# halajun/diasss

Measured on AMD Instinct MI355X. Metric: sonar frames/sec end-to-end (extract+match+LM solve), higher is better.
Workload: dtype u8/int32 (extract, match) + f64 (geo gate, LM); 1 GPU; 200 synthetic 2000x1024 frames, dense all-pairs; frames=200, pings=2000, bins=1024, pairs=19900

## Files before the change

diasss_amd/csrc/dsss_pg.hip:

```cpp
#include "dsss_internal.h"
#include "dsss_lm.h"
#include <utility>
#include "dsss_pg_kernels.h"
#include <algorithm>
#include <numeric>
#include <random>
#include <cstdlib>
#include <chrono>
#include <thread>
#include <mutex>
#include <future>

namespace {

struct pg_dev {
    dsss_ctx* ctx = nullptr;
    int rc = DSSS_OK;
    static constexpr size_t CHUNK = (size_t)256 << 20;
    template <typename T> int alloc(dsss_ctx* c, T** p, size_t n) { void* q = nullptr; if (!rc) rc = grab(c, &q, std::max<size_t>(n, 1) * sizeof(T)); *p = (T*)q; return rc; }
    int grab(dsss_ctx* c, void** p, size_t n) {
        if (!ctx) { ctx = c; c->pg_chunk_cur = 0; c->pg_chunk_off = 0; }
        const size_t bytes = (n + 255) & ~(size_t)255;
        for (;;) {
            if (c->pg_chunk_cur < c->pg_chunks.size()) {
// ... 541 lines not shown
        for (const pg_sched* H : { &A.SO, &A.SI })
            for (int l = 0; l < H->nlev; ++l) {
                const int nit = H->lv_ptr[l + 1] - H->lv_ptr[l];
                if (nit > 0) c->pg_last_levels.insert(c->pg_last_levels.end(), { nit, H->max_w6[l], H->max_rows[l], H == &A.SI ? 1 : 0 });
            }
        dv.alloc(c, &d_Tinv, (size_t)std::max(S.npanels, 1) * PG_NB4 * 16);
        size_t need = 0;
        for (const pg_sched* H : { &A.SO, &A.SI })
            for (int l = 0; l < H->nlev; ++l)
                if (64 * H->trsm_chunks[l] > PG_BWD_SPLIT) need = std::max(need, (size_t)(H->lv_ptr[l + 1] - H->lv_ptr[l]) * ((64 * H->trsm_chunks[l] + PG_BWD_RC - 1) / PG_BWD_RC) * 96);
        if ((need > 0 && dv.alloc(c, &d_bwp, need)) || dv.rc) return dv.rc;
        bwd_lds = (int)(((PG_PW * 6) * PG_BWD2_LD + PG_NB4 * 16 + 10 * (PG_PW * 6) + std::min(max_n6, PG_BWD2_SX) + 16) * sizeof(double));
        if (bwd_lds > 160 * 1024) DSSS_FAIL(c, DSSS_E_CAPACITY, "front of %d scalar rows: back-substitution needs %d B of LDS", max_n6, bwd_lds);
        hipFuncSetAttribute((const void*)pg_front_bwd2_kernel, hipFuncAttributeMaxDynamicSharedMemorySize, 160 * 1024);
        (void)hipGetLastError();
        return DSSS_OK;
    }

    void run_levels(const pg_sched& H, const dsched& Dv, int part = 0) {
        for (int l = 0; l < H.nlev; ++l) {
            const int nas = part == 2 ? 0 : H.asmrow_ptr[l + 1] - H.asmrow_ptr[l], nit = part == 1 ? 0 : H.lv_ptr[l + 1] - H.lv_ptr[l], ntl = H.tile_ptr[l + 1] - H.tile_ptr[l];
            const int* itf = Dv.lv_front + H.lv_ptr[l]; const int* its = Dv.lv_step + H.lv_ptr[l];
            if (nas > 0) { dsss_scope s2(c, DSSS_K_PG_ASM);
                hipLaunchKernelGGL(pg_front_asm_kernel, dim3(nas), dim3(256), 0, st, Dv.asm_front + H.asmrow_ptr[l], Dv.asm_row + H.asmrow_ptr[l], d_FD, d_CH, d_rel, d_xr_ptr, d_xr_child, d_xr_row,
                                   d_fa_rowptr, d_fa_src, d_fa_col, d_fa_tr, d_aval, d_x, d_F, d_R); }
            if (nit == 0) continue;
            { dsss_scope s3(c, DSSS_K_PG_DIAG, H.fl_diag[l]);
              hipLaunchKernelGGL(pg_front_diag4_kernel, dim3(nit), dim3(256), 0, st, itf, its, d_FD, d_F, d_R, d_fail, d_Tinv); }
            if (ntl > 0 && ntl <= PG_RSU_MAX_TILES) {
                dsss_scope s45(c, DSSS_K_PG_RSU, H.fl_trsm[l] + H.fl_syrk[l]);
                if (ntl <= PG_RSU32_MAX_TILES)
                    hipLaunchKernelGGL(pg_front_rsu_kernel<32>, dim3(4 * ntl), dim3(256), 0, st, itf, its, d_FD, Dv.tile_item + H.tile_ptr[l], Dv.tile_ij + H.tile_ptr[l], d_F, d_FL, d_R, d_Tinv);
                else hipLaunchKernelGGL(pg_front_rsu_kernel<64>, dim3(ntl), dim3(512), 0, st, itf, its, d_FD, Dv.tile_item + H.tile_ptr[l], Dv.tile_ij + H.tile_ptr[l], d_F, d_FL, d_R, d_Tinv);
            } else if (H.trsm_chunks[l] > 0) {
                { dsss_scope s4(c, DSSS_K_PG_TRSM, H.fl_trsm[l]);
                  hipLaunchKernelGGL(pg_front_trsm2_kernel, dim3(nit, H.trsm_chunks[l]), dim3(256), 0, st, itf, its, d_FD, d_F, d_R, d_Tinv); }
                { dsss_scope s5(c, DSSS_K_PG_ACC, H.fl_syrk[l]);
                  if (ntl > 0) hipLaunchKernelGGL(pg_front_syrk_kernel, dim3(ntl), dim3(256), 0, st, itf, its, d_FD, Dv.tile_item + H.tile_ptr[l], Dv.tile_ij + H.tile_ptr[l], d_F); }
            }
        }
    }
    void run_levels_bwd(const pg_sched& H, const dsched& Dv) {
        for (int l = H.nlev - 1; l >= 0; --l) {
            const int nit = H.lv_ptr[l + 1] - H.lv_ptr[l];
            if (nit == 0) continue;
            dsss_scope s6(c, DSSS_K_PG_BWD, H.fl_bwd[l], 2);
            const int ntl = H.tile_ptr[l + 1] - H.tile_ptr[l];
            const double* Fl = (ntl > 0 && ntl <= PG_RSU_MAX_TILES) ? d_FL : d_F;
// ... 388 lines not shown
```

diasss_amd/csrc/dsss_pg_fronts.hip:

```cpp
#include "dsss_pg_kernels.h"
#include "dsss_pg_dev.h"
#include <utility>
#pragma clang fp contract(fast)

__global__ __launch_bounds__(256) void pg_front_asm_kernel(const int* __restrict__ it_front, const int* __restrict__ it_row, const pg_front* __restrict__ FD,
                                                           const pg_child* __restrict__ CH, const int* __restrict__ rel, const int* __restrict__ xr_ptr,
                                                           const int* __restrict__ xr_child, const int* __restrict__ xr_row, const int* __restrict__ fa_rowptr,
                                                           const int* __restrict__ fa_src, const int* __restrict__ fa_col, const int* __restrict__ fa_tr,
                                                           const double* __restrict__ aval, const double* __restrict__ x, double* __restrict__ F, double* __restrict__ R)
{
    const pg_front fd = FD[it_front[blockIdx.x]];
    const int Rb = it_row[blockIdx.x], ld = fd.ld;
    double* __restrict__ A = F + fd.off + (size_t)(6 * Rb) * ld; double* __restrict__ r = R + fd.roff + 6 * Rb;
    const int ncol = 6 * (Rb + 1);
    for (int cc = threadIdx.x; cc < ncol; cc += 256) {
#pragma unroll
        for (int a = 0; a < 6; ++a) A[(size_t)a * ld + cc] = 0.0;
    }
    if (threadIdx.x < 6) { const int i = 6 * Rb + threadIdx.x; r[threadIdx.x] = i < fd.s6 ? x[(size_t)fd.c0 * 6 + i] : 0.0; }
    __syncthreads();
    {
        const int lo = fa_rowptr[fd.rowptr + Rb], hi = fa_rowptr[fd.rowptr + Rb + 1];
        const int grp = threadIdx.x / 36, el = threadIdx.x % 36;
        if (grp < 7)
            for (int e = lo + grp; e < hi; e += 7) {
                if (e > lo && fa_col[e - 1] == fa_col[e]) continue;
                const int a = el / 6, b = el % 6;
                double v = 0;
                for (int e2 = e; e2 < hi && fa_col[e2] == fa_col[e]; ++e2) v += aval[(size_t)fa_src[e2] * 36 + (fa_tr[e2] ? b * 6 + a : a * 6 + b)];
                A[(size_t)a * ld + fa_col[e] * 6 + b] += v;
            }
    }
    __syncthreads();
    const int q_lo = xr_ptr[fd.rowptr + Rb], q_hi = xr_ptr[fd.rowptr + Rb + 1];
    pg_child cd_n = {}; int i_n = 0;
    if (q_lo < q_hi) { cd_n = CH[xr_child[q_lo]]; i_n = xr_row[q_lo]; }
    for (int q = q_lo; q < q_hi; ++q) {
// ... 88 lines not shown
#pragma unroll
        for (int u = 0; u < 12; ++u) {
            const int e = threadIdx.x + 256 * u, rr = e / 48, c2 = e - 48 * rr;
            *reinterpret_cast<double2*>(&sB[rr * PG_SYRK_LD + 2 * c2]) = v[u];
        }
    }
    const int i0 = 64 * ti + 16 * wave;
    const int ir = i0 + (l & 15);
    double a[24];
    pg_d4 acc[4];
    {
        const double* __restrict__ Ai = A + (size_t)(P.row0 + min(ir, nrows - 1)) * ld + P.col0;
#pragma unroll
        for (int ks = 0; ks < 24; ++ks) { const int k = 4 * ks + (l >> 4); a[ks] = (ir < nrows && k < n) ? Ai[k] : 0.0; }
        pg_strip_load<64>(acc, A, P, true, i0, tj, l);
    }
#pragma unroll
    for (int ks = 0; ks < 24; ++ks) a[ks] = -a[ks];
    __syncthreads();
    if (i0 >= nrows) return;
    pg_strip_update<64>(acc, [&](int ks) { return a[ks]; }, sB, A, P, i0, tj, l);
}

#define PG_LDS_BARRIER() do { asm volatile("s_waitcnt lgkmcnt(0)" ::: "memory"); __builtin_amdgcn_s_barrier(); asm volatile("" ::: "memory"); } while (0)
struct pg_d4_lds { double lp[3][7][64]; double li[2][16]; int bad; };
struct pg_lag_desc { int kind, I, T2; };
constexpr pg_lag_desc pg_lag_get(int W, int NT, int R, int want)
{
    const int I0 = W, I1 = W + 4, K = 4 * NT;
    const bool act0 = I0 < NT, act1 = I1 < 7 && (I1 < NT || I1 == 6);
    int idx = 0;
    if (R >= 2) {
        const int k = R - 2, t = k / 4, b = k % 4;
        const bool piv = (t & 3) == W;
        for (int c = 0; c < 2; ++c) {
            const int I = c ? I1 : I0;
            if (!(c ? act1 : act0) || I < t) continue;
            for (int T2 = t; T2 < 6; ++T2) {
                if (T2 > I || T2 >= NT) continue;
                if (piv && T2 == t && I == t) continue;
                if (b == 3 && T2 == t + 1 && I == t + 1) continue;
                if (idx == want) return { 1, I, T2 };
                ++idx;
            }
        }
    }
    if (R >= 1 && R <= K) {
// ... 490 lines not shown
```

diasss_amd/csrc/dsss_pg_kernels.h:

```cpp
#pragma once
#include "dsss_internal.h"
#include "dsss_pose.h"
#include "dsss_pg_sym.h"

struct pg_weights { double prior[6], odo[6]; };

struct pg_level {
    int nseg, lo, hi;
    int *order, *ends;
    double *D, *g, *C, *E, *Dl, *gi, *delta;
    double *segDL, *segDR, *segGL, *segGR, *segS;
};

struct pg_pack { const double* U; const double* g; double* dst; int cld, cb; };
struct pg_front {
    long long off, roff;
    int ld, n6, s6, c0;
    int rowptr, pan0;
    int ch0, ch1, fa0, fa1;
};
struct pg_child { const double* U; const double* g; long long relptr; int cld, cb; };

#define PG_ASM_POSES 32
#define PG_NB4 24
#define PG_RSU_MAX_TILES 320
#define PG_RSU32_MAX_TILES 80
#define PG_BWD2_LD 97
#define PG_BWD2_SX 8192
#define PG_BWD_SPLIT 2048
#define PG_BWD_RC 512
#define RNG_PER_THREAD 16

template <bool WJ> __global__ void pg_linearize_kernel(int n, int ne, const pose_t* __restrict__ X, const pose_t* __restrict__ meas, pg_weights W, const int* __restrict__ ea, const int* __restrict__ eb, const int* __restrict__ eo, const pose_t* __restrict__ emeas, const double* __restrict__ ew, double* __restrict__ r, double* __restrict__ Ji, double* __restrict__ partial, int mp0, int mp1);
__global__ void pg_final_sum_kernel(const double* __restrict__ partial, int n, double scale, double* __restrict__ out);
__global__ void pg_assemble_kernel(int n, pg_weights W, const double* __restrict__ r, const double* __restrict__ Ji, const int* __restrict__ adj_ptr, const int* __restrict__ adj_edge, const double* __restrict__ ew, const double* __restrict__ lambda_ptr, double* __restrict__ D, double* __restrict__ C, double* __restrict__ g, const int* __restrict__ eo, int mp0, int mp1, const int* __restrict__ plist, int np);
template <bool FROMJ> __global__ void pg_segment_kernel(pg_level lv, int* __restrict__ fail, const double* __restrict__ rf, const double* __restrict__ Jf, pg_weights W, const double* __restrict__ lambda_ptr);
__global__ void pg_chain1_kernel(pg_level lv0, pg_level lv1);
__global__ void pg_scatter_base_kernel(pg_level lv, const int* __restrict__ perm, const int* __restrict__ dest, double* __restrict__ Lvals, double* __restrict__ aval, double* __restrict__ rhs, const int* __restrict__ if_slot, double* __restrict__ aval_if, double* __restrict__ x_if);
__global__ void pg_scatter_lc_kernel(int n, int ne, int ns, const double* __restrict__ Ji, const double* __restrict__ ew, const int* __restrict__ dest, double* __restrict__ Lvals, double* __restrict__ aval, double* __restrict__ aval_if, const int* __restrict__ eo, int mp0, int mp1, const int* __restrict__ lc_link);
__global__ void pg_comm_pack_kernel(const int* __restrict__ it_child, const int* __restrict__ it_row, const pg_pack* __restrict__ PK);
__global__ void pg_comm_xif_kernel(int nif, const int* __restrict__ if_sep, const int* __restrict__ perm, const double* __restrict__ x_if, double* __restrict__ x);
__global__ void pg_comm_scal_kernel(const double* __restrict__ scal, const int* __restrict__ fail, double* __restrict__ red);
__global__ void pg_sep_delta_kernel(pg_level lv, const int* __restrict__ perm, const double* __restrict__ x);
template <bool FROMJ> __global__ void pg_backsub_kernel(pg_level lv, const double* __restrict__ Jf, pg_weights W);
__global__ void pg_linerr_kernel(int n, int ne, pg_weights W, const int* __restrict__ ea, const int* __restrict__ eb, const int* __restrict__ eo, const double* __restrict__ ew, const double* __restrict__ r, const double* __restrict__ Ji, const double* __restrict__ delta, double* __restrict__ partial, int mp0, int mp1);
__global__ void pg_retract_kernel(int n, const pose_t* __restrict__ X, const double* __restrict__ delta, pose_t* __restrict__ Xn);
// ... 3 lines not shown
__global__ void pg_flag_compact_kernel(const int* __restrict__ flags, const double* __restrict__ pairs, long long n, const int* __restrict__ bsum, long long need_pairs, double* __restrict__ normals);
__global__ void lc_edge_compact_kernel(const int* __restrict__ flags, const int* __restrict__ bsum, const unsigned long long* __restrict__ slot, int total, const int* __restrict__ kp7_off, const double* __restrict__ kp7,
                                       const dsss_lc* __restrict__ lcs, const int* __restrict__ act_s, const int* __restrict__ frame_off, int cap, dsss_lc_edge* __restrict__ edges, int2* __restrict__ ab);
__global__ void pg_gather_dr_kernel(const unsigned long long* __restrict__ fptr, const int* __restrict__ foff, double* __restrict__ out);
__global__ void pg_gather_pose_kernel(int n, const int* __restrict__ idx, const pose_t* __restrict__ X, pose_t* __restrict__ out);
__global__ void pg_sep_xy_kernel(int ns, const int* __restrict__ sep_pose, const double* __restrict__ dr6, double* __restrict__ xy);
__global__ void pg_init_kernel(int n, const double* __restrict__ dr6, const double* __restrict__ normals, int add_noise, pose_t* __restrict__ X, pose_t* __restrict__ meas);
__global__ void pg_rpy_kernel(int n, const pose_t* __restrict__ X, double* __restrict__ rpy6);
__global__ void pg_build_map_kernel(int nupd, const int* __restrict__ rlrow, const int* __restrict__ rlptr, const int* __restrict__ rlcol, const int* __restrict__ rlpos, const int* __restrict__ colptr, const int* __restrict__ rowidx, const long long* __restrict__ mapptr, int* __restrict__ upd_map, const int* __restrict__ nupd_dev);
__global__ void pg_rl_count_kernel(int ns, const int* __restrict__ colptr, const int* __restrict__ rowidx, const char* __restrict__ binned, int* __restrict__ cnt);
template <typename T, int VAL>
__global__ void pg_scan_block_kernel(int n, const int* __restrict__ cnt, const int* __restrict__ colptr, T* __restrict__ out, T* __restrict__ block_sum);
template <typename T>
__global__ void pg_scan_tops_kernel(int nblocks, T* __restrict__ block_sum, T* __restrict__ total);
template <typename T>
__global__ void pg_scan_add_kernel(int n, T* __restrict__ out, const T* __restrict__ block_sum, const T* __restrict__ total);
__global__ void pg_rl_fill_kernel(int ns, const int* __restrict__ colptr, const int* __restrict__ rowidx, const char* __restrict__ binned, const int* __restrict__ rlptr, int* __restrict__ cur, int* __restrict__ rlcol, int* __restrict__ rlpos);
__global__ void pg_rl_sort_kernel(int ns, const int* __restrict__ rlptr, int* __restrict__ rlcol, int* __restrict__ rlpos, int* __restrict__ rlrow, int* __restrict__ fail);
__global__ void pg_fill_map_kernel(int* __restrict__ upd_map, const long long* __restrict__ total);
__global__ void pg_anc_rel_kernel(int ns, const int* __restrict__ colptr, const int* __restrict__ rowidx, const char* __restrict__ binned, const int* __restrict__ root_of, int* __restrict__ anc_first, int* __restrict__ anc_rel);
__global__ void pg_factor_subtree_kernel(const int* __restrict__ bin_perm, const int* __restrict__ binptr, const int* __restrict__ bincols, const int* __restrict__ colptr, const int* __restrict__ rlptr, const int* __restrict__ rlcol, const int* __restrict__ rlpos, const long long* __restrict__ mapptr, const int* __restrict__ upd_map, double* __restrict__ Lvals, double* __restrict__ x, int* __restrict__ fail, const int* __restrict__ binroot_ptr, const int* __restrict__ binroot_idx, const int* __restrict__ broot_b, const long long* __restrict__ broot_uoff, const int* __restrict__ broot_of_col, const int* __restrict__ anc_first, const int* __restrict__ anc_rel, double* __restrict__ ubin, double* __restrict__ rdiag);
__global__ void pg_factor_subtree_serial_kernel(const int* __restrict__ bin_perm, const int* __restrict__ binptr, const int* __restrict__ bincols, const int* __restrict__ colptr, const int* __restrict__ rlptr, const int* __restrict__ rlcol, const int* __restrict__ rlpos, const long long* __restrict__ mapptr, const int* __restrict__ upd_map, double* __restrict__ Lvals, double* __restrict__ x, int* __restrict__ fail, const int* __restrict__ binroot_ptr, const int* __restrict__ binroot_idx, const int* __restrict__ broot_b, const long long* __restrict__ broot_uoff, const int* __restrict__ broot_of_col, const int* __restrict__ anc_first, const int* __restrict__ anc_rel, double* __restrict__ ubin, double* __restrict__ rdiag);
__global__ void pg_bwd_subtree_kernel(const int* __restrict__ bin_perm, const int* __restrict__ binptr, const int* __restrict__ bincols, const int* __restrict__ colptr, const int* __restrict__ rowidx, const double* __restrict__ Lvals, double* __restrict__ x, const double* __restrict__ rdiag);
__global__ void pg_front_asm_kernel(const int* __restrict__ it_front, const int* __restrict__ it_row, const pg_front* __restrict__ FD, const pg_child* __restrict__ CH, const int* __restrict__ rel, const int* __restrict__ xr_ptr, const int* __restrict__ xr_child, const int* __restrict__ xr_row, const int* __restrict__ fa_rowptr, const int* __restrict__ fa_src, const int* __restrict__ fa_col, const int* __restrict__ fa_tr, const double* __restrict__ aval, const double* __restrict__ x, double* __restrict__ F, double* __restrict__ R);
__global__ void pg_front_syrk_kernel(const int* __restrict__ it_front, const int* __restrict__ it_step, const pg_front* __restrict__ FD, const int* __restrict__ tile_item, const int* __restrict__ tile_ij, double* __restrict__ F);
__global__ void pg_front_diag4_kernel(const int* __restrict__ it_front, const int* __restrict__ it_step, const pg_front* __restrict__ FD, double* __restrict__ F, double* __restrict__ R, int* __restrict__ fail, double* __restrict__ Tinv);
__global__ void pg_front_trsm2_kernel(const int* __restrict__ it_front, const int* __restrict__ it_step, const pg_front* __restrict__ FD, double* __restrict__ F, double* __restrict__ R, const double* __restrict__ Tinv);
template <int TS>
__global__ void pg_front_rsu_kernel(const int* __restrict__ it_front, const int* __restrict__ it_step, const pg_front* __restrict__ FD, const int* __restrict__ tile_item, const int* __restrict__ tile_ij, double* __restrict__ F, double* __restrict__ FL, double* __restrict__ R, const double* __restrict__ Tinv);
__global__ void pg_front_bwd_part_kernel(const int* __restrict__ it_front, const int* __restrict__ it_step, const pg_front* __restrict__ FD, const int* __restrict__ f_rows, const double* __restrict__ FL, const double* __restrict__ x, double* __restrict__ part, int maxchunks);
__global__ void pg_front_bwd2_kernel(const int* __restrict__ it_front, const int* __restrict__ it_step, const pg_front* __restrict__ FD, const int* __restrict__ f_rows, const double* __restrict__ F, const double* __restrict__ FL, const double* __restrict__ R, double* __restrict__ x, const double* __restrict__ Tinv, const double* __restrict__ part, int maxchunks);
```

diasss_amd/csrc/dsss_pg_sym.cpp:

```cpp
#include "dsss_pg_sym.h"
#include <algorithm>
#include <atomic>
#include <chrono>
#include <condition_variable>
#include <deque>
#include <functional>
#include <cmath>
#include <cstdio>
#include <cstdlib>
#include <cstring>
#include <mutex>
#include <numeric>
#include <thread>

namespace {

class pg_pool {
public:
    struct task { std::function<void()> fn; std::atomic<int> st{ 0 }; };
    static pg_pool& get() { static pg_pool P; return P; }
    void fork(task* t)
    {
        if (workers.empty()) { t->st.store(1); t->fn(); t->st.store(2, std::memory_order_release); return; }
        { std::lock_guard<std::mutex> lk(mu); q.push_back(t); npending.fetch_add(1, std::memory_order_release); }
// ... 841 lines not shown
        for (int f = 0; f < nf; ++f) if (S.f_n[f] > 100) ++big;
        fprintf(stderr, "[dsss pg symbolic] adjacency %.2f + ND %.2f ms, column structures %.1f ms, bins+lists %.1f ms, fronts+schedule %.1f ms | ns %d nnzL %lld bins %d (%zu cols, %zu roots, U %.1f MB) fronts %d (>100 rows: %d, max %d) panels %d levels %d front arena %.1f MB comm %.1f MB front GFLOP %.1f (column count %.1f)\n",
                ms(t_start, t_adj), ms(t_adj, t_order), ms(t_order, t_cols), ms(t_cols, t_fork), ms_since(t_fork), ns, S.nnzL, (int)S.binptr.size() - 1, S.bincols.size(), S.broot.size(), S.ubin_doubles * 8e-6,
                nf, big, S.max_front_n, S.npanels, S.nlev, S.front_doubles * 8e-6, S.comm_doubles * 8e-6, S.flops_fronts * 1e-9, S.flops_factor * 1e-9);
    }
};
void pg_symbolic(int ns, const std::vector<std::pair<int, int>>& edges, const double* cx, const double* cy, const int* part, int nparts,
                 const pg_sym_opts& opt, pg_sym& S)
{
    sym_run R(ns, edges, cx, cy, part, nparts, opt, S);
    R.adjacency();
    if (opt.before_order) opt.before_order();
    R.tp[sym_run::t_adj] = sym_run::clock::now();
    R.order(); R.columns(); R.bins();
    R.supernodes(); R.children(); R.entries(); R.schedule(); R.interface(); R.finish();
}
void pg_build_schedule(const pg_sym& S, int part_lo, int part_hi, pg_sched& out)
{
    out = pg_sched();
    out.nlev = S.nlev;
    const int nl = S.nlev;
    out.lv_ptr.assign(nl + 1, 0); out.asmrow_ptr.assign(nl + 1, 0); out.tile_ptr.assign(nl + 1, 0);
    out.trsm_chunks.assign(nl, 0); out.fl_diag.assign(nl, 0); out.fl_trsm.assign(nl, 0); out.fl_syrk.assign(nl, 0); out.fl_bwd.assign(nl, 0);
    out.max_w6.assign(nl, 0); out.max_rows.assign(nl, 0);
    auto sel = [&](int f) { return S.f_part[f] >= part_lo && S.f_part[f] < part_hi; };
    {
        size_t nrow = 0, nitem = 0, ntile = 0;
        for (size_t f = 0; f < S.f_c0.size(); ++f) {
            if (!sel((int)f)) continue;
            nrow += (size_t)S.f_n[f]; nitem += (size_t)S.f_npan[f];
            for (int k = 0; k < S.f_npan[f]; ++k) { const int n6 = 6 * S.f_n[f], w6 = std::min(96, 6 * S.f_s[f] - 96 * k), nt = (n6 - 96 * k - w6 + 63) / 64; ntile += (size_t)nt * (nt + 1) / 2; }
        }
        out.asmrow_front.reserve(nrow); out.asmrow_row.reserve(nrow); out.lv_front.reserve(nitem); out.lv_step.reserve(nitem); out.tile_item.reserve(ntile); out.tile_ij.reserve(ntile);
    }
    for (int l = 0; l < nl; ++l) {
        for (int q = S.asm_ptr[l]; q < S.asm_ptr[l + 1]; ++q) { const int f = S.asm_front[q]; if (!sel(f)) continue; for (int r = 0; r < S.f_n[f]; ++r) { out.asmrow_front.push_back(f); out.asmrow_row.push_back(r); } }
        out.asmrow_ptr[l + 1] = (int)out.asmrow_front.size();
        for (int q = S.lv_ptr[l]; q < S.lv_ptr[l + 1]; ++q) {
            const int f = S.lv_front[q], k = S.lv_step[q];
            if (!sel(f)) continue;
            const int item = (int)out.lv_front.size() - out.lv_ptr[l];
            out.lv_front.push_back(f); out.lv_step.push_back(k);
            const int n6 = 6 * S.f_n[f], w6 = std::min(96, 6 * S.f_s[f] - 96 * k), nrows = n6 - 96 * k - w6, nt = (nrows + 63) / 64;
            for (int ti = 0; ti < nt; ++ti) for (int tj = 0; tj <= ti; ++tj) { out.tile_item.push_back(item); out.tile_ij.push_back((ti << 16) | tj); }
            out.max_n6 = std::max(out.max_n6, n6);
            out.max_w6[l] = std::max(out.max_w6[l], w6); out.max_rows[l] = std::max(out.max_rows[l], nrows);
            out.trsm_chunks[l] = std::max(out.trsm_chunks[l], (nrows + 63) / 64);
            const double nn = w6, rows = nrows;
            out.fl_diag[l] += nn * nn * nn / 3.0 + nn * nn; out.fl_trsm[l] += rows * nn * nn; out.fl_bwd[l] += 2.0 * rows * nn + nn * nn; out.fl_syrk[l] += rows * (rows + 1) * nn;
        }
        out.lv_ptr[l + 1] = (int)out.lv_front.size(); out.tile_ptr[l + 1] = (int)out.tile_item.size();
    }
}

int h_chol(double* A, int n, int ld)
{
    for (int j = 0; j < n; ++j) {
        double d = A[(size_t)j * ld + j];
        for (int k = 0; k < j; ++k) d -= A[(size_t)j * ld + k] * A[(size_t)j * ld + k];
// ... 297 lines not shown
    sym_levels(G);
    sym_row_views(G, std::max(1, opt.threads));
    if (tv) { fprintf(stderr, "[dsss pg symbolic] separators per part:"); for (auto& q : P) fprintf(stderr, " %d", q.nint); fprintf(stderr, "\n"); }
    if (tv) fprintf(stderr, "[dsss pg symbolic] %d parts + an interface of %d: interface %.2f ms, the parts (their graphs, the wait for the coordinates, the analyses; largest %d separators) %.2f ms, joined %.2f ms, levels and row views %.2f ms | ns %d nnzL %lld bins %d fronts %d (max %d rows) panels %d levels %d front arena %.1f MB\n",
                    K, nif, t_pre, [&] { int m = 0; for (auto& q : P) m = std::max(m, q.g.size()); return m; }(), t_parts - t_pre, t_join - t_parts, ms_since(q0) - t_join, ns, G.nnzL,
                    nbG, nfG, G.max_front_n, G.npanels, G.nlev, G.front_doubles * 8e-6);
    return true;
}

}

pg_switches pg_switches_read()
{
    pg_switches sw;
    if (const char* v = getenv("DSSS_PG_BIN_COST")) sw.bin_cost = sw.opt.bin_cost = atof(v);
    if (const char* v = getenv("DSSS_PG_LEAF")) sw.opt.leaf = atoi(v);
    if (const char* v = getenv("DSSS_PG_ND_BOTH")) sw.opt.nd_both_axes = atoi(v);
    if (const char* v = getenv("DSSS_PG_ND_INDEX")) sw.opt.nd_index_cuts = atoi(v);
    if (const char* v = getenv("DSSS_PG_PARTS_ANALYSIS")) sw.parts = atoi(v);
    if (const char* v = getenv("DSSS_SYM_THREADS")) sw.threads = atoi(v);
    if (const char* v = getenv("DSSS_PG_LOCAL")) sw.local = atoi(v) != 0;
    if (const char* v = getenv("DSSS_PG_VERBOSE")) sw.opt.verbose = std::max(1, atoi(v));
    if (const char* v = getenv("DSSS_PG_BINS")) sw.bins_serial = strcmp(v, "serial") == 0;
    return sw;
}
int pg_cheapest_gap(const int* pos, const std::vector<int>& cross, int target, int width, int after, int* cost)
{
    const int m = (int)cross.size() - 1, lo = std::max(target - width, after + 1);
    auto start = [&](int i) { return pos ? pos[i - 1] + 1 : i; };
    int best = -1; long long bdist = 0;
    for (int i = std::max(1, pos ? (int)(std::lower_bound(pos, pos + m, lo - 1) - pos) + 1 : lo); i < m && start(i) <= target + width; ++i) {
        const long long d = std::llabs((long long)start(i) - target);
        if (best < 0 || cross[i] < *cost || (cross[i] == *cost && d < bdist)) { *cost = cross[i]; bdist = d; best = start(i); }
    }
    return best;
}

void pg_analyse(int ns, const std::vector<std::pair<int, int>>& edges, const double* cx, const double* cy, const int* part, int nparts,
                int part_lo, int part_hi, int world, int rank, const pg_switches& sw, pg_sym_opts opt, pg_analysis& A)
{
    auto sym_threads = [&](int m) { return sw.threads && *sw.threads > 0 ? *sw.threads : (int)std::min(m >= 131072 ? 24u : 8u, std::max(1u, std::thread::hardware_concurrency())); };
    opt.bin_cost = sw.bin_cost.value_or(PG_BIN_COST_DEVICE);
    opt.threads = sym_threads(ns);
    pg_sym& S = A.S;
    if (world > 1 && sw.local) {
        std::vector<int> rank_of_part(nparts, 0), rank_of(ns);
// ... 104 lines not shown
    p[0] = nb; p[1] = (int64_t)S.bincols.size();
    for (int b = 0; b < nb; ++b) {
        const int lo = S.binptr[b], hi = S.binptr[b + 1];
        if (hi - lo == 1) ++p[2];
        p[8] = std::max<int64_t>(p[8], S.binroot_ptr[b + 1] - S.binroot_ptr[b]);
        p[10] = std::max<int64_t>(p[10], hi - lo);
        for (int ci = lo; ci < hi; ++ci) {
            const int j = S.bincols[ci], T = S.rlptr[j + 1] - S.rlptr[j], m = S.colptr[j + 1] - S.colptr[j];
            bool fresh = false;
            if (ci > lo) {
                const int jp = S.bincols[ci - 1], Tp = S.rlptr[jp + 1] - S.rlptr[jp];
                fresh = T > 0 && S.rlcol[S.rlptr[j + 1] - 1] == jp;
                if (T == 0 && Tp > 0) ++p[3];
                if (fresh) ++p[4]; else if (T > 0) ++p[5];
                if (S.broot_of_col[j] >= 0 && S.broot_of_col[j] == S.broot_of_col[jp] && m - S.anc_first[j] > 0 && S.colptr[jp + 1] - S.colptr[jp] - S.anc_first[jp] > 0) ++p[9];
            }
            p[6] = std::max<int64_t>(p[6], T - (fresh ? 1 : 0));
            p[7] = std::max<int64_t>(p[7], m);
            p[11] = std::max<int64_t>(p[11], T);
        }
    }
    return DSSS_OK;
}
extern "C" int dsss_host_pg_solve_local(int ns, const int32_t* edge_a, const int32_t* edge_b, int nedges, const double* cx, const double* cy,
                                        const int32_t* iface_last, int nlast, const double* aval, const double* rhs, double* x, int64_t* stats8)
{
    if (ns < 1 || nedges < 0 || (nedges > 0 && (!edge_a || !edge_b)) || !cx || !cy || nlast < 0 || nlast > ns || (nlast > 0 && !iface_last) || !x || !aval || !rhs) return DSSS_E_ARG;
    std::vector<std::pair<int, int>> edges;
    if (!twin_edges(ns, edge_a, edge_b, nedges, false, false, edges)) return DSSS_E_ARG;
    pg_sym S; pg_sym_opts opt = pg_switches_read().opt;
    for (int q = 0; q < nlast; ++q) {
        if (iface_last[q] < 0 || iface_last[q] >= ns || (q > 0 && iface_last[q] <= iface_last[q - 1])) return DSSS_E_ARG;
        opt.iface_last.push_back(iface_last[q]);
    }
    pg_symbolic(ns, edges, cx, cy, nullptr, 1, opt, S);
    if (nlast > 0) {
        const int nf = (int)S.f_c0.size();
        if (!iface_front_last(S, nlast)) return DSSS_E_STATE;
        for (int f = 0; f + 1 < nf; ++f) if (S.f_part[f] < 0) return DSSS_E_STATE;
        for (int q = 0; q < nlast; ++q) if (S.order[ns - nlast + q] != iface_last[q] || (int)S.iface_seps.size() != nlast || S.iface_seps[q] != iface_last[q]) return DSSS_E_STATE;
        if (!S.comm_kind.empty()) return DSSS_E_STATE;
    }
    const int rc = pg_host_solve(S, aval, rhs, x);
    return twin_result(S, rc, (int64_t)S.comm_vals.size(), stats8);
}
extern "C" int dsss_host_pg_solve_parts(int ns, const int32_t* edge_a, const int32_t* edge_b, int nedges, const double* cx, const double* cy,
// ... 13 lines not shown
```

diasss_amd/csrc/dsss_pg_sym.h:

```cpp
#pragma once
#include <functional>
#include <optional>
#include <vector>

void dsss_pool_run(int T, const std::function<void(int)>& fn);

#define PG_PW 16
#define PG_PARTS_CUT_MAX 12
#define PG_PARTS_IFACE_MAX 256
#define PG_LOCAL_IFACE_MAX 160

constexpr double PG_BIN_COST_HOST = 1000, PG_BIN_COST_DEVICE = 600, PG_BIN_COST_RANK = 120;

struct pg_sym {
    int ns = 0, nparts = 1;
    std::vector<int> perm;
    std::vector<int> order;
    std::vector<int> colptr, rowidx;
    std::vector<int> parent;
    std::vector<int> col_part;
    std::vector<char> binned;
    std::vector<int> binptr, bincols;
    std::vector<int> bin_part;
    std::vector<double> bin_work;
// ... 20 lines not shown
    long long front_doubles = 0, frhs_doubles = 0;
    std::vector<int> ch_ptr, ch_kind, ch_id;
    std::vector<long long> ch_relptr;
    std::vector<int> rel;
    std::vector<int> fa_ptr, fa_src, fa_row, fa_col, fa_tr;
    std::vector<int> dest_bin;
    std::vector<int> fa_rowptr, xr_ptr, xr_child, xr_row;
    int nlev = 0, npanels = 0;
    std::vector<int> lv_ptr, lv_front, lv_step;
    std::vector<int> asm_ptr, asm_front;
    std::vector<int> comm_kind, comm_id, comm_part;
    std::vector<long long> comm_off;
    long long comm_doubles = 0;
    std::vector<int> comm_vals, iface_seps;
    int nval = 0;
    double flops_factor = 0, flops_fronts = 0; long long nnzL = 0; int max_front_n = 0;
    int ownership_violations = 0;
};

struct pg_sched {
    int nlev = 0;
    std::vector<int> lv_ptr, lv_front, lv_step;
    std::vector<int> asmrow_ptr, asmrow_front, asmrow_row;
    std::vector<int> tile_ptr, tile_item, tile_ij;
    std::vector<int> trsm_chunks;
    std::vector<double> fl_diag, fl_trsm, fl_syrk, fl_bwd;
    std::vector<int> max_w6, max_rows;
    int max_n6 = 6;
};

struct pg_sym_opts {
    int leaf = 24;
    int nd_both_axes = 64;
    int nd_index_cuts = 1;
    bool nd_geo_first = true;
    double bin_cost = PG_BIN_COST_HOST;
    double pack_cost = 0;
    int threads = 4;
    double relax_zero_blocks = 8, relax_flops = 1.05, relax_flops_small = 1.6;
    double relax_abs_flops = 0;
    std::function<void()> on_bottom_ready;
    std::function<void()> on_lists_ready;
    bool lists_on_device = false;
    std::function<void()> before_order;
    std::vector<int> iface_last;
    bool to_be_joined = false;
    int verbose = 0;
};

struct pg_switches {
    pg_sym_opts opt;
    std::optional<double> bin_cost;
    std::optional<int> parts, threads;
    bool local = true;
    bool bins_serial = false;
};
pg_switches pg_switches_read();

int pg_cheapest_gap(const int* pos, const std::vector<int>& cross, int target, int width, int after, int* cost);

struct pg_analysis {
    pg_sym S;
    pg_sched SO, SI;
    bool local = false;
    std::vector<int> perm_g, dest_g, ifslot_g, ifsep_g;
};
void pg_analyse(int ns, const std::vector<std::pair<int, int>>& edges, const double* cx, const double* cy, const int* part, int nparts,
                int part_lo, int part_hi, int world, int rank, const pg_switches& sw, pg_sym_opts opt, pg_analysis& A);
```

include/dsss.h:

```cpp
#ifndef DSSS_H
#define DSSS_H

#include <stdint.h>
#include <stddef.h>

#ifdef __cplusplus
extern "C" {
#endif

#define DSSS_OK            0
#define DSSS_E_NODEVICE   -1
#define DSSS_E_ARG        -2
#define DSSS_E_HIP        -3
#define DSSS_E_STATE      -4
#define DSSS_E_CAPACITY   -5
#define DSSS_E_NUMERIC    -6
#define DSSS_E_COMM       -7

typedef struct dsss_ctx dsss_ctx;

typedef struct { float x, y, size, angle, response; int32_t octave; } dsss_kp;

typedef struct {
    double factor;  int32_t width, r, side;
// ... 95 lines not shown
int dsss_posegraph_update_window(dsss_ctx*, int nframes, int window_frames, double* poses12_host, double* rpy6_host, double* stats4_host);
int dsss_posegraph_reset(dsss_ctx*);
int dsss_posegraph_online_edges(dsss_ctx*);
int dsss_posegraph_schedule_get(dsss_ctx*, int* levels4_host, int cap_levels, int* n_levels, int* n_trials);
int dsss_posegraph_solve_edges(dsss_ctx*, const double* dr6, int total, const dsss_lc_edge* edges, int ne,
                               double* poses12_host, double* stats4_host);

int dsss_posegraph_edge_report(dsss_ctx*, const double* dr6, int total, const dsss_lc_edge* edges, int ne,
                               const double* poses12, double* chi2_host, double* r6_host, double* sums3_host);

typedef struct { double gate, decade; int32_t max_solves, pad_; } dsss_pg_gate_params;
void dsss_pg_gate_params_default(dsss_pg_gate_params*);
int dsss_posegraph_solve_gated(dsss_ctx*, const double* dr6, int total, const dsss_lc_edge* edges, int ne,
                               const dsss_pg_gate_params*, double* poses12_host, double* stats4_host,
                               uint8_t* keep_host , double* chi2_host , int* n_solves_host);

int dsss_host_pg_solve(int ns, const int32_t* edge_a, const int32_t* edge_b, int nedges, const double* cx, const double* cy,
                       const int32_t* part, int nparts, const double* aval36, const double* rhs6, double* x6_host, int64_t* stats8);
int dsss_host_pg_solve_local(int ns, const int32_t* edge_a, const int32_t* edge_b, int nedges, const double* cx, const double* cy,
                             const int32_t* iface_last, int nlast, const double* aval36, const double* rhs6, double* x6_host, int64_t* stats8);
int dsss_host_pg_solve_parts(int ns, const int32_t* edge_a, const int32_t* edge_b, int nedges, const double* cx, const double* cy,
                             int K, const double* aval36, const double* rhs6, double* x6_host, int64_t* stats8);
int dsss_host_pg_bins_profile(int ns, const int32_t* edge_a, const int32_t* edge_b, int nedges, const double* cx, const double* cy, int64_t* prof12);

typedef struct { double x0, y0, cell; int32_t W, H; int32_t use_mask; int32_t pad_; } dsss_mosaic_params;
int dsss_mosaic_grid(const double* bbox4, double cell, dsss_mosaic_params* out);
int dsss_mosaic_bounds(dsss_ctx*, const int* ids, int n, const double* rpy6, const int* ping_off, double* bbox4_host);
int dsss_mosaic_render(dsss_ctx*, const int* ids, int n, const double* rpy6, const int* ping_off,
                       const dsss_mosaic_params*, uint32_t* sum_host, uint32_t* cnt_host, uint8_t* img_host);
int dsss_mosaic_consistency(dsss_ctx*, const int* ids, int n, const double* rpy6, const int* ping_off,
                            const dsss_mosaic_params*, uint32_t* nfr_host, uint32_t* s1_host, uint32_t* s2_host,
                            double* score_host);

typedef struct { int32_t min_count, smooth, target, pad_; } dsss_gain_params;
void dsss_gain_params_default(dsss_gain_params*);
int  dsss_mosaic_gain_stats(dsss_ctx*, const int* ids, int n, int use_mask, uint64_t* sum_host , uint64_t* cnt_host );
int  dsss_mosaic_gain_table(const uint64_t* sum, const uint64_t* cnt, int M, const dsss_gain_params* ,
                            uint16_t* gain_q8 , int32_t* target_out );
int  dsss_mosaic_gain_set(dsss_ctx*, const uint16_t* gain_q8_host, int M);
int  dsss_mosaic_gain_get(dsss_ctx*, uint16_t* gain_q8_host, int cap, int* M);

#define DSSS_COMP_NEAR  0
#define DSSS_COMP_FAR   1
#define DSSS_COMP_MID   2
#define DSSS_COMP_FIRST 3
typedef struct { int32_t mode, fill_radius; } dsss_comp_params;
// ... 106 lines not shown
```

Baseline: 9829 frames/s.

## Assemble pose-graph front rows in LDS with prefetched child contributions

Adds an LDS path to the front assembly kernel. Each 6-row block is zeroed, has its original entries and child extend-add updates accumulated in shared memory, and is written to the global front once. Child update rows are prefetched into registers in batches of four so global loads overlap with the LDS accumulation. The goal is to remove repeated global read-modify-write traffic on F. The cost is dynamic LDS use of up to 1344 columns × 6 doubles per block and extra barriers. A global fallback remains available through an environment switch, along with a host profiling helper.

```diff
diff --git a/diasss_amd/csrc/dsss_pg.hip b/diasss_amd/csrc/dsss_pg.hip
--- a/diasss_amd/csrc/dsss_pg.hip
+++ b/diasss_amd/csrc/dsss_pg.hip
@@ -587,8 +587,9 @@
             const int nas = part == 2 ? 0 : H.asmrow_ptr[l + 1] - H.asmrow_ptr[l], nit = part == 1 ? 0 : H.lv_ptr[l + 1] - H.lv_ptr[l], ntl = H.tile_ptr[l + 1] - H.tile_ptr[l];
             const int* itf = Dv.lv_front + H.lv_ptr[l]; const int* its = Dv.lv_step + H.lv_ptr[l];
             if (nas > 0) { dsss_scope s2(c, DSSS_K_PG_ASM);
-                hipLaunchKernelGGL(pg_front_asm_kernel, dim3(nas), dim3(256), 0, st, Dv.asm_front + H.asmrow_ptr[l], Dv.asm_row + H.asmrow_ptr[l], d_FD, d_CH, d_rel, d_xr_ptr, d_xr_child, d_xr_row,
-                                   d_fa_rowptr, d_fa_src, d_fa_col, d_fa_tr, d_aval, d_x, d_F, d_R); }
+                const int lds_cols = sw.asm_global ? 0 : std::min(H.asm_cols[l], PG_ASM_LDS_COLS);
+                hipLaunchKernelGGL(pg_front_asm_kernel, dim3(nas), dim3(256), (size_t)lds_cols * 6 * sizeof(double), st, Dv.asm_front + H.asmrow_ptr[l], Dv.asm_row + H.asmrow_ptr[l], d_FD, d_CH, d_rel, d_xr_ptr, d_xr_child, d_xr_row,
+                                   d_fa_rowptr, d_fa_src, d_fa_col, d_fa_tr, d_aval, d_x, d_F, d_R, lds_cols); }
             if (nit == 0) continue;
             { dsss_scope s3(c, DSSS_K_PG_DIAG, H.fl_diag[l]);
               hipLaunchKernelGGL(pg_front_diag4_kernel, dim3(nit), dim3(256), 0, st, itf, its, d_FD, d_F, d_R, d_fail, d_Tinv); }
diff --git a/diasss_amd/csrc/dsss_pg_fronts.hip b/diasss_amd/csrc/dsss_pg_fronts.hip
--- a/diasss_amd/csrc/dsss_pg_fronts.hip
+++ b/diasss_amd/csrc/dsss_pg_fronts.hip
@@ -3,16 +3,108 @@
 #include <utility>
 #pragma clang fp contract(fast)
 
+#define PG_LDS_BARRIER() do { asm volatile("s_waitcnt lgkmcnt(0)" ::: "memory"); __builtin_amdgcn_s_barrier(); asm volatile("" ::: "memory"); } while (0)
+
+__device__ __forceinline__ void pg_asm_row_lds(const pg_front fd, const int Rb, double* sA, const pg_child* __restrict__ CH, const int* __restrict__ rel, const int* __restrict__ xr_ptr,
+                                               const int* __restrict__ xr_child, const int* __restrict__ xr_row, const int* __restrict__ fa_rowptr,
+                                               const int* __restrict__ fa_src, const int* __restrict__ fa_col, const int* __restrict__ fa_tr,
+                                               const double* __restrict__ aval, const double* __restrict__ x, double* __restrict__ F, double* __restrict__ R)
+{
+    const int ld = fd.ld, ncol = 6 * (Rb + 1), tid = threadIdx.x;
+    const int lo = fa_rowptr[fd.rowptr + Rb], hi = fa_rowptr[fd.rowptr + Rb + 1];
+    const int q_lo = xr_ptr[fd.rowptr + Rb], q_hi = xr_ptr[fd.rowptr + Rb + 1];
+    double rv = 0.0;
+    if (tid < 6) { const int i = 6 * Rb + tid; rv = i < fd.s6 ? x[(size_t)fd.c0 * 6 + i] : 0.0; }
+    for (int cc = tid; cc < 6 * ncol; cc += 256) sA[cc] = 0.0;
+    PG_LDS_BARRIER();
+    pg_child cd[PG_ASM_PF] = {}; int ci[PG_ASM_PF] = {};
+    int rlv[PG_ASM_PF]; double u[PG_ASM_PF][6], g[PG_ASM_PF];
+    auto records = [&](int q0) {
+#pragma unroll
+        for (int p = 0; p < PG_ASM_PF; ++p) if (q0 + p < q_hi) { cd[p] = CH[xr_child[q0 + p]]; ci[p] = xr_row[q0 + p]; }
+    };
+    auto request = [&](int q0) {
+#pragma unroll
+        for (int p = 0; p < PG_ASM_PF; ++p) {
+            rlv[p] = 0; g[p] = 0.0;
+#pragma unroll
+            for (int a = 0; a < 6; ++a) u[p][a] = 0.0;
+            if (q0 + p < q_hi) {
+                const int i = ci[p];
+                if (tid < 6 * (i + 1)) {
+                    const double* __restrict__ src = cd[p].U + (size_t)(6 * i) * cd[p].cld + tid;
+                    rlv[p] = rel[cd[p].relptr + tid / 6];
+#pragma unroll
+                    for (int a = 0; a < 6; ++a) u[p][a] = src[(size_t)a * cd[p].cld];
+                }
+                if (tid < 6) g[p] = cd[p].g[6 * i + tid];
+            }
+        }
+    };
+    records(q_lo);
+    request(q_lo);
+    {
+        const int grp = tid / 36, el = tid % 36;
+        if (grp < 7)
+            for (int e = lo + grp; e < hi; e += 7) {
+                if (e > lo && fa_col[e - 1] == fa_col[e]) continue;
+                const int a = el / 6, b = el % 6;
+                double v = 0;
+                for (int e2 = e; e2 < hi && fa_col[e2] == fa_col[e]; ++e2) v += aval[(size_t)fa_src[e2] * 36 + (fa_tr[e2] ? b * 6 + a : a * 6 + b)];
+                sA[a * ncol + fa_col[e] * 6 + b] += v;
+            }
+    }
+    PG_LDS_BARRIER();
+    for (int q0 = q_lo; q0 < q_hi; q0 += PG_ASM_PF) {
+#pragma unroll
+        for (int p = 0; p < PG_ASM_PF; ++p) {
+            if (q0 + p >= q_hi) break;
+            const int i = ci[p], wcols = 6 * (i + 1);
+            if (tid < wcols) {
+                const int dcol = 6 * rlv[p] + tid % 6;
+#pragma unroll
+                for (int a = 0; a < 6; ++a) sA[a * ncol + dcol] = sA[a * ncol + dcol] + u[p][a];
+            }
+            if (wcols > 256) {
+                const int* __restrict__ rl = rel + cd[p].relptr;
+                const double* __restrict__ src = cd[p].U + (size_t)(6 * i) * cd[p].cld;
+                for (int cc = tid + 256; cc < wcols; cc += 256) {
+                    const int j2 = cc / 6, dcol = 6 * rl[j2] + (cc - 6 * j2);
+                    double w[6];
+#pragma unroll
+                    for (int a = 0; a < 6; ++a) w[a] = src[(size_t)a * cd[p].cld + cc];
+#pragma unroll
+                    for (int a = 0; a < 6; ++a) sA[a * ncol + dcol] = sA[a * ncol + dcol] + w[a];
+                }
+            }
+            if (tid < 6) rv += g[p];
+            PG_LDS_BARRIER();
+        }
+        if (q0 + PG_ASM_PF < q_hi) { records(q0 + PG_ASM_PF); request(q0 + PG_ASM_PF); }
+    }
+    double* __restrict__ A = F + fd.off + (size_t)(6 * Rb) * ld;
+    for (int cc = tid; cc < ncol; cc += 256) {
+#pragma unroll
+        for (int a = 0; a < 6; ++a) A[(size_t)a * ld + cc] = sA[a * ncol + cc];
+    }
+    if (tid < 6) R[fd.roff + 6 * Rb + tid] = rv;
+}
 __global__ __launch_bounds__(256) void pg_front_asm_kernel(const int* __restrict__ it_front, const int* __restrict__ it_row, const pg_front* __restrict__ FD,
                                                            const pg_child* __restrict__ CH, const int* __restrict__ rel, const int* __restrict__ xr_ptr,
                                                            const int* __restrict__ xr_child, const int* __restrict__ xr_row, const int* __restrict__ fa_rowptr,
                                                            const int* __restrict__ fa_src, const int* __restrict__ fa_col, const int* __restrict__ fa_tr,
-                                                           const double* __restrict__ aval, const double* __restrict__ x, double* __restrict__ F, double* __restrict__ R)
-{
+                                                           const double* __restrict__ aval, const double* __restrict__ x, double* __restrict__ F, double* __restrict__ R,
+                                                           int lds_cols)
+{
+    extern __shared__ __attribute__((aligned(16))) double s_asm[];
     const pg_front fd = FD[it_front[blockIdx.x]];
     const int Rb = it_row[blockIdx.x], ld = fd.ld;
+    const int ncol = 6 * (Rb + 1);
+    if (ncol <= lds_cols) {
+        pg_asm_row_lds(fd, Rb, s_asm, CH, rel, xr_ptr, xr_child, xr_row, fa_rowptr, fa_src, fa_col, fa_tr, aval, x, F, R);
+        return;
+    }
     double* __restrict__ A = F + fd.off + (size_t)(6 * Rb) * ld; double* __restrict__ r = R + fd.roff + 6 * Rb;
-    const int ncol = 6 * (Rb + 1);
     for (int cc = threadIdx.x; cc < ncol; cc += 256) {
 #pragma unroll
         for (int a = 0; a < 6; ++a) A[(size_t)a * ld + cc] = 0.0;
@@ -147,7 +239,6 @@
     pg_strip_update<64>(acc, [&](int ks) { return a[ks]; }, sB, A, P, i0, tj, l);
 }
 
-#define PG_LDS_BARRIER() do { asm volatile("s_waitcnt lgkmcnt(0)" ::: "memory"); __builtin_amdgcn_s_barrier(); asm volatile("" ::: "memory"); } while (0)
 struct pg_d4_lds { double lp[3][7][64]; double li[2][16]; int bad; };
 struct pg_lag_desc { int kind, I, T2; };
 constexpr pg_lag_desc pg_lag_get(int W, int NT, int R, int want)
diff --git a/diasss_amd/csrc/dsss_pg_kernels.h b/diasss_amd/csrc/dsss_pg_kernels.h
--- a/diasss_amd/csrc/dsss_pg_kernels.h
+++ b/diasss_amd/csrc/dsss_pg_kernels.h
@@ -22,6 +22,8 @@
 struct pg_child { const double* U; const double* g; long long relptr; int cld, cb; };
 
 #define PG_ASM_POSES 32
+#define PG_ASM_LDS_COLS 1344
+#define PG_ASM_PF 4
 #define PG_NB4 24
 #define PG_RSU_MAX_TILES 320
 #define PG_RSU32_MAX_TILES 80
@@ -71,7 +73,7 @@
 __global__ void pg_factor_subtree_kernel(const int* __restrict__ bin_perm, const int* __restrict__ binptr, const int* __restrict__ bincols, const int* __restrict__ colptr, const int* __restrict__ rlptr, const int* __restrict__ rlcol, const int* __restrict__ rlpos, const long long* __restrict__ mapptr, const int* __restrict__ upd_map, double* __restrict__ Lvals, double* __restrict__ x, int* __restrict__ fail, const int* __restrict__ binroot_ptr, const int* __restrict__ binroot_idx, const int* __restrict__ broot_b, const long long* __restrict__ broot_uoff, const int* __restrict__ broot_of_col, const int* __restrict__ anc_first, const int* __restrict__ anc_rel, double* __restrict__ ubin, double* __restrict__ rdiag);
 __global__ void pg_factor_subtree_serial_kernel(const int* __restrict__ bin_perm, const int* __restrict__ binptr, const int* __restrict__ bincols, const int* __restrict__ colptr, const int* __restrict__ rlptr, const int* __restrict__ rlcol, const int* __restrict__ rlpos, const long long* __restrict__ mapptr, const int* __restrict__ upd_map, double* __restrict__ Lvals, double* __restrict__ x, int* __restrict__ fail, const int* __restrict__ binroot_ptr, const int* __restrict__ binroot_idx, const int* __restrict__ broot_b, const long long* __restrict__ broot_uoff, const int* __restrict__ broot_of_col, const int* __restrict__ anc_first, const int* __restrict__ anc_rel, double* __restrict__ ubin, double* __restrict__ rdiag);
 __global__ void pg_bwd_subtree_kernel(const int* __restrict__ bin_perm, const int* __restrict__ binptr, const int* __restrict__ bincols, const int* __restrict__ colptr, const int* __restrict__ rowidx, const double* __restrict__ Lvals, double* __restrict__ x, const double* __restrict__ rdiag);
-__global__ void pg_front_asm_kernel(const int* __restrict__ it_front, const int* __restrict__ it_row, const pg_front* __restrict__ FD, const pg_child* __restrict__ CH, const int* __restrict__ rel, const int* __restrict__ xr_ptr, const int* __restrict__ xr_child, const int* __restrict__ xr_row, const int* __restrict__ fa_rowptr, const int* __restrict__ fa_src, const int* __restrict__ fa_col, const int* __restrict__ fa_tr, const double* __restrict__ aval, const double* __restrict__ x, double* __restrict__ F, double* __restrict__ R);
+__global__ void pg_front_asm_kernel(const int* __restrict__ it_front, const int* __restrict__ it_row, const pg_front* __restrict__ FD, const pg_child* __restrict__ CH, const int* __restrict__ rel, const int* __restrict__ xr_ptr, const int* __restrict__ xr_child, const int* __restrict__ xr_row, const int* __restrict__ fa_rowptr, const int* __restrict__ fa_src, const int* __restrict__ fa_col, const int* __restrict__ fa_tr, const double* __restrict__ aval, const double* __restrict__ x, double* __restrict__ F, double* __restrict__ R, int lds_cols);
 __global__ void pg_front_syrk_kernel(const int* __restrict__ it_front, const int* __restrict__ it_step, const pg_front* __restrict__ FD, const int* __restrict__ tile_item, const int* __restrict__ tile_ij, double* __restrict__ F);
 __global__ void pg_front_diag4_kernel(const int* __restrict__ it_front, const int* __restrict__ it_step, const pg_front* __restrict__ FD, double* __restrict__ F, double* __restrict__ R, int* __restrict__ fail, double* __restrict__ Tinv);
 __global__ void pg_front_trsm2_kernel(const int* __restrict__ it_front, const int* __restrict__ it_step, const pg_front* __restrict__ FD, double* __restrict__ F, double* __restrict__ R, const double* __restrict__ Tinv);
diff --git a/diasss_amd/csrc/dsss_pg_sym.cpp b/diasss_amd/csrc/dsss_pg_sym.cpp
--- a/diasss_amd/csrc/dsss_pg_sym.cpp
+++ b/diasss_amd/csrc/dsss_pg_sym.cpp
@@ -887,7 +887,7 @@
     const int nl = S.nlev;
     out.lv_ptr.assign(nl + 1, 0); out.asmrow_ptr.assign(nl + 1, 0); out.tile_ptr.assign(nl + 1, 0);
     out.trsm_chunks.assign(nl, 0); out.fl_diag.assign(nl, 0); out.fl_trsm.assign(nl, 0); out.fl_syrk.assign(nl, 0); out.fl_bwd.assign(nl, 0);
-    out.max_w6.assign(nl, 0); out.max_rows.assign(nl, 0);
+    out.max_w6.assign(nl, 0); out.max_rows.assign(nl, 0); out.asm_cols.assign(nl, 0);
     auto sel = [&](int f) { return S.f_part[f] >= part_lo && S.f_part[f] < part_hi; };
     {
         size_t nrow = 0, nitem = 0, ntile = 0;
@@ -899,7 +899,7 @@
         out.asmrow_front.reserve(nrow); out.asmrow_row.reserve(nrow); out.lv_front.reserve(nitem); out.lv_step.reserve(nitem); out.tile_item.reserve(ntile); out.tile_ij.reserve(ntile);
     }
     for (int l = 0; l < nl; ++l) {
-        for (int q = S.asm_ptr[l]; q < S.asm_ptr[l + 1]; ++q) { const int f = S.asm_front[q]; if (!sel(f)) continue; for (int r = 0; r < S.f_n[f]; ++r) { out.asmrow_front.push_back(f); out.asmrow_row.push_back(r); } }
+        for (int q = S.asm_ptr[l]; q < S.asm_ptr[l + 1]; ++q) { const int f = S.asm_front[q]; if (!sel(f)) continue; out.asm_cols[l] = std::max(out.asm_cols[l], 6 * S.f_n[f]); for (int r = 0; r < S.f_n[f]; ++r) { out.asmrow_front.push_back(f); out.asmrow_row.push_back(r); } }
         out.asmrow_ptr[l + 1] = (int)out.asmrow_front.size();
         for (int q = S.lv_ptr[l]; q < S.lv_ptr[l + 1]; ++q) {
             const int f = S.lv_front[q], k = S.lv_step[q];
@@ -1243,6 +1243,7 @@
     if (const char* v = getenv("DSSS_PG_LOCAL")) sw.local = atoi(v) != 0;
     if (const char* v = getenv("DSSS_PG_VERBOSE")) sw.opt.verbose = std::max(1, atoi(v));
     if (const char* v = getenv("DSSS_PG_BINS")) sw.bins_serial = strcmp(v, "serial") == 0;
+    if (const char* v = getenv("DSSS_PG_ASM")) sw.asm_global = strcmp(v, "global") == 0;
     return sw;
 }
 int pg_cheapest_gap(const int* pos, const std::vector<int>& cross, int target, int width, int after, int* cost)
@@ -1393,6 +1394,38 @@
     }
     return DSSS_OK;
 }
+extern "C" int dsss_host_pg_asm_profile(int ns, const int32_t* edge_a, const int32_t* edge_b, int nedges, const double* cx, const double* cy, int lds_cols_max, int pf, int64_t* prof8)
+{
+    if (ns < 1 || nedges < ns - 1 || !edge_a || !edge_b || !cx || !cy || !prof8) return DSSS_E_ARG;
+    std::vector<std::pair<int, int>> edges;
+    if (!twin_edges(ns, edge_a, edge_b, nedges, true, true, edges)) return DSSS_E_ARG;
+    pg_sym S;
+    const pg_switches sw = pg_switches_read();
+    pg_sym_opts opt = sw.opt;
+    if (sw.threads) opt.threads = std::max(1, *sw.threads);
+    opt.bin_cost = sw.bin_cost.value_or(PG_BIN_COST_DEVICE);
+    pg_symbolic(ns, edges, cx, cy, nullptr, 1, opt, S);
+    pg_sched H; pg_build_schedule(S, 0, 1, H);
+    int64_t* p = prof8;
+    for (int k = 0; k < 8; ++k) p[k] = 0;
+    p[0] = (int64_t)H.asmrow_front.size();
+    for (int l = 0; l < H.nlev; ++l) {
+        int widest = 0;
+        for (int q = H.asmrow_ptr[l]; q < H.asmrow_ptr[l + 1]; ++q) {
+            const int f = H.asmrow_front[q], Rb = H.asmrow_row[q], ncol = 6 * (Rb + 1);
+            widest = std::max(widest, ncol);
+            if (ncol > lds_cols_max) ++p[2];
+            const int q_lo = S.xr_ptr[S.f_rowptr[f] + Rb], q_hi = S.xr_ptr[S.f_rowptr[f] + Rb + 1];
+            p[3] = std::max<int64_t>(p[3], q_hi - q_lo);
+            if (q_hi == q_lo) ++p[5];
+            if (q_hi - q_lo > pf) ++p[6];
+            for (int q2 = q_lo; q2 < q_hi; ++q2) p[4] = std::max<int64_t>(p[4], 6 * (S.xr_row[q2] + 1));
+        }
+        p[1] = std::max<int64_t>(p[1], widest);
+        if (widest != H.asm_cols[l]) ++p[7];
+    }
+    return DSSS_OK;
+}
 extern "C" int dsss_host_pg_solve_local(int ns, const int32_t* edge_a, const int32_t* edge_b, int nedges, const double* cx, const double* cy,
                                         const int32_t* iface_last, int nlast, const double* aval, const double* rhs, double* x, int64_t* stats8)
 {
diff --git a/diasss_amd/csrc/dsss_pg_sym.h b/diasss_amd/csrc/dsss_pg_sym.h
--- a/diasss_amd/csrc/dsss_pg_sym.h
+++ b/diasss_amd/csrc/dsss_pg_sym.h
@@ -66,6 +66,7 @@
     int nlev = 0;
     std::vector<int> lv_ptr, lv_front, lv_step;
     std::vector<int> asmrow_ptr, asmrow_front, asmrow_row;
+    std::vector<int> asm_cols;
     std::vector<int> tile_ptr, tile_item, tile_ij;
     std::vector<int> trsm_chunks;
     std::vector<double> fl_diag, fl_trsm, fl_syrk, fl_bwd;
@@ -98,6 +99,7 @@
     std::optional<int> parts, threads;
     bool local = true;
     bool bins_serial = false;
+    bool asm_global = false;
 };
 pg_switches pg_switches_read();
 
diff --git a/include/dsss.h b/include/dsss.h
--- a/include/dsss.h
+++ b/include/dsss.h
@@ -141,6 +141,7 @@
 int dsss_host_pg_solve_parts(int ns, const int32_t* edge_a, const int32_t* edge_b, int nedges, const double* cx, const double* cy,
                              int K, const double* aval36, const double* rhs6, double* x6_host, int64_t* stats8);
 int dsss_host_pg_bins_profile(int ns, const int32_t* edge_a, const int32_t* edge_b, int nedges, const double* cx, const double* cy, int64_t* prof12);
+int dsss_host_pg_asm_profile(int ns, const int32_t* edge_a, const int32_t* edge_b, int nedges, const double* cx, const double* cy, int lds_cols_max, int pf, int64_t* prof8);
 
 typedef struct { double x0, y0, cell; int32_t W, H; int32_t use_mask; int32_t pad_; } dsss_mosaic_params;
 int dsss_mosaic_grid(const double* bbox4, double cell, dsss_mosaic_params* out);
```

New measurement: 9785 frames/s. No clear change (-0.4%).
